# happyjin/Gaussian_process

Measured on AMD Instinct MI355X. Metric: GP-fit+predict sec and achieved fp64 TFLOP/s, N=65536 d=8, 1/2/4/8 MI355X, higher is better.
Workload: dtype f64; 1 GPU; GP fit+predict N=65536 d=8 n_test=4096 (BASELINE configs[2]); N=65536, d=8, n_test=4096, partition=single GPU

## Files before the change

### gaussian_process_amd/_lib.py

```python
from __future__ import annotations

import ctypes as C
import os

import numpy as np


_HERE = os.path.dirname(os.path.abspath(__file__))
LIB_PATH = os.path.join(_HERE, "libgpmi355x.so")

GPMI_OK, GPMI_ERR_NOT_PD, GPMI_ERR_BAD_ARG, GPMI_ERR_RUNTIME = 0, 1, 2, 3
ABI_VERSION = 4
SOFTMAX_MAX_CLASSES = 10
SPARSE_METHODS = {"vfe": 0, "fitc": 1}

T_KBUILD, T_CHOL, T_CHOL_PANEL, T_CHOL_TRAIL, T_LML, T_KS, T_SOLVE_V, T_MEANVAR, \
    T_ALPHA, T_POSTCHOL, T_TRAIL_LAUNCHES, T_TRAIL_FLOPS = range(12)
T_COUNT = 16
TIMER_NAMES = ["kbuild", "chol", "chol_panel", "chol_trail", "lml", "ks", "solve_v", "meanvar",
               "alpha", "postchol", "trail_launches", "trail_flops", "grad", "loo", "sparse"]

_dp = C.POINTER(C.c_double)
_i64 = C.c_int64
_vp = C.c_void_p

SIGNATURES = {
    "gpmi_abi_version": [],
    "gpmi_device_count": [C.POINTER(C.c_int)],
    "gpmi_ctx_create": [C.c_int, C.POINTER(_vp)],
    "gpmi_ctx_destroy": [_vp],
    "gpmi_set_option": [_vp, C.c_char_p, _i64],
    "gpmi_rbf": [_vp, _dp, _i64, _dp, _i64, _i64, C.c_double, C.c_double, _dp],
    "gpmi_cov": [_vp, C.c_int, _dp, _i64, _dp, _i64, _i64, C.c_double, C.c_double, _dp],
    "gpmi_set_kernel": [_vp, C.c_int, C.c_double, C.c_double],
    "gpmi_cov_params": [_vp, C.c_int, _dp, _i64, _dp, _i64, _i64, _dp, C.c_int, _dp],
    "gpmi_set_kernel_params": [_vp, C.c_int, _dp, C.c_int],
    "gpmi_set_train": [_vp, _dp, _i64, _i64, _dp],
    "gpmi_factorize": [_vp, C.c_double, C.c_double, C.c_double, _dp, C.POINTER(_i64)],
    "gpmi_fit": [_vp, _dp, _i64, _i64, _dp, C.c_double, C.c_double, C.c_double, _dp, C.POINTER(_i64)],
    "gpmi_append": [_vp, _dp, _i64, _dp, _dp, C.POINTER(_i64)],
    "gpmi_remove": [_vp, C.POINTER(_i64), _i64, _dp],
    "gpmi_get_layout": [_vp, C.POINTER(_i64)],
    "gpmi_get_alpha": [_vp, _dp],
    "gpmi_get_m": [_vp, _dp],
    "gpmi_get_diag": [_vp, _dp],
    "gpmi_get_factor_block": [_vp, _i64, _i64, _i64, _i64, _dp],
    "gpmi_set_test": [_vp, _dp, _i64],
    "gpmi_predict_resident": [_vp, _dp, _dp, C.c_int],
    "gpmi_predict": [_vp, _dp, _i64, _dp, _dp, C.c_int],
    "gpmi_fit_predict_resident": [_vp, C.c_double, C.c_double, C.c_double, _dp, C.POINTER(_i64), _dp, _dp, C.c_int],
    "gpmi_fit_predict_sample_resident": [_vp, C.c_double, C.c_double, C.c_double, C.c_double, _dp, C.POINTER(_i64), _dp, _dp,
                                         C.c_int, _dp],
    "gpmi_post_chol": [_vp, C.c_double, _dp, C.POINTER(_i64)],
    "gpmi_post_sample": [_vp, C.c_double, _dp, _i64, _dp, C.POINTER(_i64)],
    "gpmi_lml_grad": [_vp, _dp, _dp],
    "gpmi_set_lengthscales": [_vp, _dp, _i64],
    "gpmi_lml_grad_ard": [_vp, _dp, _dp, _dp, _dp],
    "gpmi_lml_grad_co2": [_vp, _dp, _dp],
    "gpmi_loo": [_vp, _dp, _dp, _dp, _dp],
    "gpmi_loo_grad": [_vp, _dp, _dp, _dp],
    "gpmi_grad_trace": [_vp, _dp, _dp, _i64, _i64, C.c_double, C.c_double, _dp, _dp, _dp, _dp],
    "gpmi_lml_batch": [_vp, _dp, _i64, _dp, C.POINTER(C.c_int)],
    "gpmi_laplace_fit": [_vp, C.c_double, C.c_double, C.c_double, C.c_int, _dp, C.POINTER(C.c_int), C.POINTER(C.c_int), _dp],
    "gpmi_laplace_predict_resident": [_vp, _dp, _dp, _dp],
    "gpmi_laplace_grad": [_vp, _dp, _dp, _dp],
# ... 118 lines not shown
```

### gaussian_process_amd/csrc/driver.hip

```cpp
#include "gpmi_ctx.h"
#include "gpmi_plan.h"

namespace gpmi {

hipError_t panel_rec(hipStream_t s, double* A, int64_t ld, int64_t mrows, int64_t off, int64_t w,
                     int64_t col_offset, int64_t* info) {
    hipError_t e;
    const bool fused = tuning().panel_fused && w % 128 == 0 && off % 128 == 0;
    const int64_t leaf = fused ? 128 : IB;
    if (w <= leaf) {
        double* Ajj = A + off * ld + off;
        const int64_t below = mrows - off - leaf;
        if (fused) {
            if ((e = launch_potrf128(s, Ajj, ld, col_offset + off, info)) != hipSuccess) return e;
            if (below > 0) return launch_trsm128(s, Ajj, ld, A + (off + leaf) * ld + off, ld, below);
            return hipSuccess;
        }
        if ((e = launch_potf2_64(s, Ajj, ld, col_offset + off, info)) != hipSuccess) return e;
        if (below > 0) return launch_trsm_rlt64(s, Ajj, ld, A + (off + IB) * ld + off, ld, below);
        return hipSuccess;
    }
    const int64_t h = (w / 2) / leaf * leaf;
    if ((e = panel_rec(s, A, ld, mrows, off, h, col_offset, info)) != hipSuccess) return e;
    {
// ... 12 lines not shown
}

hipError_t trsm_rec(hipStream_t s, const double* L, int64_t ldl, double* X, int64_t ldx, int64_t m,
                    int64_t off, int64_t w) {
    hipError_t e;
    const bool fused = tuning().panel_fused && w % 128 == 0 && off % 128 == 0 && m % 128 == 0;
    const int64_t leaf = fused ? 128 : IB;
    if (w <= leaf) {
        if (fused) return launch_trsm128(s, L + off * ldl + off, ldl, X + off, ldx, m);
        return launch_trsm_rlt64(s, L + off * ldl + off, ldl, X + off, ldx, m);
    }
    const int64_t h = (w / 2) / leaf * leaf;
    if ((e = trsm_rec(s, L, ldl, X, ldx, m, off, h)) != hipSuccess) return e;
    const GemmArgs g = gemm_minus(X + off + h, ldx, X + off, ldx, L + (off + h) * ldl + off, ldl, m, w - h, h);
    if ((e = launch_gemm_nt(s, g)) != hipSuccess) return e;
    return trsm_rec(s, L, ldl, X, ldx, m, off + h, w - h);
}

hipError_t trsm_block(hipStream_t s, const double* L, int64_t ldl, double* X, int64_t ldx,
                      int64_t m, int64_t nb) {
    return trsm_rec(s, L, ldl, X, ldx, m, 0, nb);
}

hipError_t cholesky_inplace(gpmi_ctx* c, double* A, int64_t ld, int64_t ncols, int64_t nrows,
                            int64_t* info, bool account, int64_t carried_rows) {
    hipError_t e;
    hipStream_t sm = c->stream;
    const int64_t NB = c->block(ncols);
    const bool la = c->lookahead_for(ncols);
    hipStream_t sp_ = la ? c->pstream : sm;
    const bool slack = la && ncols >= 49152;
    SharingScope shallow(la ? Sharing::beside_update().with_panel_slack(slack) : sharing());
    const int slot_p = account ? GPMI_T_CHOL_PANEL : GPMI_T_COUNT - 1;
    const int slot_t = account ? GPMI_T_CHOL_TRAIL : GPMI_T_COUNT - 1;
    if (la && (e = c->order(sm, sp_)) != hipSuccess) return e;
    auto trail = [&](hipStream_t st, bool counted, int64_t r0, int64_t c0, int64_t k, int64_t nb, int64_t ncol_upd) -> hipError_t {
        GemmArgs g = gemm_minus_lower(A + r0 * ld + c0, ld, A + r0 * ld + k, ld, A + c0 * ld + k, ld, nrows - r0, ncol_upd,
                                      nb, r0 - c0);
        g.role = counted ? 1 : 0;
        const GemmRoute route = gemm_nt_route(g);
        const bool dma = gemm_kernel_is_dma(route.kernel);
        size_t sp = c->span_begin(counted ? (dma ? slot_t : GPMI_T_COUNT - 1) : slot_p, st);
        hipError_t er = launch_gemm_nt(st, g, route);
        c->span_end(sp, st);
        if (account && dma && counted) {
            c->stage_ms[GPMI_T_TRAIL_LAUNCHES] += 1.0;
            c->stage_ms[GPMI_T_TRAIL_FLOPS] += gemm_nt_algorithmic_flops(g, ncols - r0 + 1 + carried_rows);
        }
        return er;
    };
    hipEvent_t ev_b = nullptr;
    for (int64_t k = 0; k < ncols; k += NB) {
        const int64_t nb = std::min<int64_t>(NB, ncols - k);
        size_t sp = c->span_begin(slot_p, sp_);
        {
            SharingScope panel_forms(!la ? sharing().large_lds()
                                     : (ncols - k >= c->shallow_min ? Sharing::beside_update() : Sharing::chip_shared_only()).with_panel_slack(slack));
            e = panel_factor(sp_, A + k * ld + k, ld, nb, nrows - k, k, info);
        }
        c->span_end(sp, sp_);
        if (e != hipSuccess) return e;
        if (la && (e = c->order(sp_, sm)) != hipSuccess) return e;
        const int64_t r0 = k + nb;
        if (r0 >= ncols) continue;
        if (!la) {
            if ((e = trail(sm, true, r0, r0, k, nb, ncols - r0)) != hipSuccess) return e;
            continue;
        }
        const int64_t nbn = std::min<int64_t>(NB, ncols - r0);
        if (ev_b && (e = hipStreamWaitEvent(sp_, ev_b, 0)) != hipSuccess) return e;
        if ((e = trail(sp_, false, r0, r0, k, nb, nbn)) != hipSuccess) return e;
        if (r0 + nbn < ncols) {
            if ((e = trail(sm, true, r0 + nbn, r0 + nbn, k, nb, ncols - r0 - nbn)) != hipSuccess) return e;
            ev_b = c->new_event();
            if (!ev_b) return c->ev_error;
            if ((e = hipEventRecord(ev_b, sm)) != hipSuccess) return e;
        }
    }
    return hipSuccess;
}

RbfArgs rbf_cross(const gpmi_ctx* c, const double* A, int64_t nA, const Box& ba, const double* B, int64_t nB, const Box& bb,
                  int64_t row0, int64_t nrows, int64_t ncols, double* out, int64_t ld) {
    RbfArgs r;
    r.A = A; r.B = B;
    r.nA = nA; r.nB = nB; r.d = c->d; r.row0 = row0; r.nrows = nrows; r.ncols = ncols;
    r.coef = c->coef; r.sig2 = c->sig2;
    r.kind = c->kind; r.kp0 = c->kp0; r.kp1 = c->kp1;
    for (int i = 0; i < 11; ++i) r.kpv[i] = c->kpv[i];
    r.diag_add = 0.; r.symmetric = 0;
    r.delta_square = (A == c->x_test() && B == c->x_train() && nA == nB) ? 1 : 0;
    r.max_sq = box_max_sq(ba, bb);
    r.out = out; r.ld = ld;
    return r;
}

RbfArgs rbf_sym(const gpmi_ctx* c, const double* X, int64_t n, const Box& box, double diag_add, int64_t npad, double* out,
                int64_t ld) {
    RbfArgs r = rbf_cross(c, X, n, box, X, n, box, 0, npad, npad, out, ld);
    r.diag_add = diag_add; r.symmetric = 1; r.delta_square = 1;
    return r;
}

RbfArgs rbf_test_train(const gpmi_ctx* c, double* out, int64_t ld) {
    return rbf_cross(c, c->x_test(), c->n, c->box_test(), c->x_train(), c->N, c->box_train(), 0, c->np_, c->Np, out, ld);
}

int ensure_train_buffers(gpmi_ctx* c, int64_t test_rows, bool test_cols) {
    c->spareA.release();
    c->Np = round_up(c->N, TILE);
    const int64_t cap = round_up(c->N + c->reserve, TILE);
    c->ldA = cap + (test_cols ? test_rows : 0) + c->ld_pad;
    c->Mp = c->Np + TILE + test_rows;
    c->rows_cap = cap + TILE + test_rows;
    c->yrow = test_cols ? c->Np + test_rows : c->Np;
    HIP_TRY(c->A.ensure((size_t)c->rows_cap * c->ldA * sizeof(double)));
    HIP_TRY(c->info.ensure(sizeof(int64_t)));
    HIP_TRY(c->red.ensure(16 * sizeof(double)));
    return GPMI_OK;
}

void meanvar_to_host(gpmi_ctx* c, const std::vector<double>& h, double* mu, double* out2, int want_sd) {
    for (int64_t i = 0; i < c->n; ++i) {
        if (mu) mu[i] = h[i];
        if (out2) {
            double kss = c->sig2;
            if (c->kind == 2) kss = 1.0;
            else if (c->kind == 3) {
                const double* th = c->kpv;
                kss = ((th[0] * th[0] + th[2] * th[2]) + th[5] * th[5]) + (th[8] * th[8] + th[10] * th[10]);
            }
            else if (c->kind == 1) {
                kss = 0.0;
                for (int64_t k = 0; k < c->d; ++k) {
                    const double e = c->hXs[(size_t)i * c->d + k] - c->kp0;
                    kss = kss + e * e;
                }
            }
            const double var = kss - h[c->np_ + i];
            out2[i] = want_sd ? std::sqrt(var) : var;
        }
    }
}

int factorize_impl(gpmi_ctx* c, double sigma, double ell, double noise_var, double* lml,
                   int64_t* bad_pivot, bool with_test, double* mu, double* out2, int want_sd, bool with_post, double jitter) {
    if (!c->res.have_train) return fail_arg("gpmi_factorize: no training set (call gpmi_set_train)");
    if (cov_stationary(c->kind) && (!(ell != 0.0) || std::isnan(ell) || std::isnan(sigma)))
        return fail_arg("gpmi_factorize: ell must be non-zero and hyper-parameters finite");
    if (std::isnan(noise_var)) return fail_arg("gpmi_factorize: noise_var is NaN");
    if (c->kind == 2 && c->d != 1) return fail_arg("gpmi_factorize: the periodic kernel is 1-D only (GP_regression.py:48)");
    if (!cov_stationary(c->kind) && c->ard())
        return fail_arg("gpmi_factorize: per-dimension lengthscales need the squared-exponential or a Matern kernel (kinds 0, 4, 5, 6)");
    if (with_post && std::isnan(jitter)) return fail_arg("gpmi_fit_predict_sample: jitter is NaN");
    c->res.drop_fit();
    c->release_sparse_grad();
    int rc = ensure_train_buffers(c, with_test ? c->np_ : 0, with_post);
    if (rc) return rc;
    hipStream_t s = c->stream;
    c->timers_reset({GPMI_T_KBUILD, GPMI_T_CHOL, GPMI_T_CHOL_PANEL, GPMI_T_CHOL_TRAIL, GPMI_T_LML,
                     GPMI_T_TRAIL_LAUNCHES, GPMI_T_TRAIL_FLOPS});
    if (with_test) c->timers_reset({GPMI_T_KS, GPMI_T_SOLVE_V, GPMI_T_MEANVAR});
    c->sig2 = sigma * sigma;
    c->coef = cov_coef(c->kind, ell);
    c->sigma = sigma; c->ell = ell; c->noise = noise_var;
    double* A = c->A.as<double>();
    const int64_t big = std::numeric_limits<int64_t>::max();
    HIP_TRY(hipMemcpyAsync(c->info.p, &big, sizeof big, hipMemcpyHostToDevice, s));

    size_t sp = c->span_begin(GPMI_T_KBUILD);
    const RbfArgs r = rbf_sym(c, c->x_train(), c->N, c->box_train(), noise_var, c->Np, A, c->ldA);
    HIP_TRY(launch_rbf(s, r));
    c->span_end(sp);
    const int64_t ncols = c->Np + (with_post ? c->np_ : 0);
    HIP_TRY(launch_fill_rows(s, c->m_row(), c->ldA, TILE, ncols, 0.0));
    HIP_TRY(launch_set_yrow(s, c->m_row(), c->y.as<double>(), c->N, c->Np));
    c->v_row0 = with_post ? c->Np : c->Np + TILE;
    double* Vr = A + c->v_row0 * c->ldA;
    if (with_test) {
        sp = c->span_begin(GPMI_T_KS);
        const RbfArgs t = rbf_test_train(c, Vr, c->ldA);
        HIP_TRY(launch_rbf(s, t));
        if (with_post) {
            const RbfArgs q = rbf_sym(c, c->x_test(), c->n, c->box_test(), jitter, c->np_, Vr + c->Np, c->ldA);
            HIP_TRY(launch_rbf(s, q));
        }
        c->span_end(sp);
    }

    sp = c->span_begin(GPMI_T_CHOL);
    HIP_TRY(cholesky_inplace(c, A, c->ldA, ncols, c->Mp, c->info.as<int64_t>(), true, with_test && !with_post ? c->n : 0));
    c->span_end(sp);

    sp = c->span_begin(GPMI_T_LML);
    HIP_TRY(launch_lml_reduce(s, A, c->ldA, c->m_row(), c->N, c->red.as<double>()));
    c->span_end(sp);

    std::vector<double> h;
    if (with_test) {
        HIP_TRY(c->vec.ensure((size_t)std::max(c->Np, c->np_) * 4 * 8));
        sp = c->span_begin(GPMI_T_MEANVAR);
        double* dot = c->vec.as<double>();
        HIP_TRY(launch_row_dots(s, Vr, c->ldA, c->np_, c->Np, c->m_row(), dot, dot + c->np_));
        c->span_end(sp);
        h.resize(2 * (size_t)c->np_);
        HIP_TRY(hipMemcpyAsync(h.data(), dot, h.size() * 8, hipMemcpyDeviceToHost, s));
    }
    double red[2];
    int64_t info;
    HIP_TRY(hipMemcpyAsync(red, c->red.p, sizeof red, hipMemcpyDeviceToHost, s));
    HIP_TRY(hipMemcpyAsync(&info, c->info.p, sizeof info, hipMemcpyDeviceToHost, s));
    HIP_TRY(hipStreamSynchronize(s));
    c->timers_collect();
    if (info != big && (info < c->N || (with_post && info >= c->Np && info < c->Np + c->n))) {
// ... 81 lines not shown
```

### gaussian_process_amd/csrc/gpmi_api.hip

```cpp
#include "gpmi_ctx.h"

using namespace gpmi;

namespace gpmi {
thread_local std::string g_err;

static thread_local Tuning t_dev_tuning;
static thread_local const Tuning* t_tuning = nullptr;
const Tuning& tuning() { return t_tuning ? *t_tuning : t_dev_tuning; }
TuneScope::TuneScope(const Tuning* t) : prev(t_tuning) { t_tuning = t; }
TuneScope::~TuneScope() { t_tuning = prev; }
static thread_local Sharing t_sharing;
Sharing& sharing() { return t_sharing; }

int ard_rescale_train(gpmi_ctx* c) {
    if (!c->ard()) return GPMI_OK;
    HIP_TRY(c->Xz.ensure((size_t)c->N * c->d * 8));
    HIP_TRY(launch_scale_inputs(c->stream, c->X.as<double>(), c->ard_rdev.as<double>(), c->N, c->d, c->Xz.as<double>()));
    HIP_TRY(hipStreamSynchronize(c->stream));
    box_scale(c->boxX, c->ard_r, c->boxZ);
    return GPMI_OK;
}
int ard_rescale_test(gpmi_ctx* c) {
    if (!c->ard()) return GPMI_OK;
// ... 37 lines not shown
    const char* env;
    if ((env = getenv("GPMI_NB"))) c->nb = std::max<int64_t>(128, atoll(env) / 128 * 128);
    if ((env = getenv("GPMI_LD_PAD"))) c->ld_pad = std::max<int64_t>(0, atoll(env) / 2 * 2);
    if ((env = getenv("GPMI_LOOKAHEAD"))) c->lookahead = atoi(env) ? 1 : 0;
    *out = c;
    return GPMI_OK;
}

int gpmi_ctx_destroy(gpmi_ctx* c) {
    if (!c) return GPMI_OK;
    for (gpmi_ctx* l : c->lane_ctx) (void)gpmi_ctx_destroy(l);
    c->lane_ctx.clear();
    (void)hipSetDevice(c->device);
    (void)hipStreamSynchronize(c->stream);
    for (DevBuf* b : {&c->X, &c->y, &c->A, &c->info, &c->red, &c->Xs, &c->V, &c->P, &c->vec, &c->dense,
                       &c->U, &c->Kn, &c->gpart, &c->cov_a, &c->cov_b, &c->cov_out, &c->flag, &c->vside,
                       &c->Xz, &c->Xsz, &c->ard_rdev, &c->gsum, &c->app, &c->spareA, &c->rem, &c->lap, &c->lap_part, &c->lap_out, &c->sm, &c->sm_part, &c->sm_E, &c->sm_B, &c->sm_out, &c->loov, &c->loow,
                       &c->sp_Zraw, &c->sp_Z, &c->sp_L, &c->sp_B, &c->sp_W, &c->sp_q, &c->sp_vec, &c->sp_part, &c->sp_scr, &c->sp_info, &c->sp_pred,
                       &c->sp_g0, &c->sp_g1, &c->sp_g2, &c->sp_gE, &c->sp_gpart, &c->sp_gvec})
        b->release();
    for (auto e : c->ev_pool) (void)hipEventDestroy(e);
    (void)hipStreamDestroy(c->stream);
    (void)hipStreamDestroy(c->pstream);
    delete c;
    return GPMI_OK;
}

static int set_tuning_option(Tuning& t, const char* name, int64_t value) {
    if (!strcmp(name, "gemm_small_tiles")) {
        t.gemm_small_tiles = value ? 1 : 0;
    } else if (!strcmp(name, "trsm_wave")) {
        t.trsm_wave = value ? 1 : 0;
    } else if (!strcmp(name, "gemm_small_dma")) {
        t.gemm_small_dma = value ? 1 : 0;
    } else if (!strcmp(name, "gemm_persist")) {
        t.gemm_persist = value ? 1 : 0;
    } else if (!strcmp(name, "gemm_ticket")) {
        if (value < 0 || value > 2) return fail_arg("gemm_ticket must be 0 (off), 1 (trailing updates under lookahead) or 2 (every launch)");
        t.gemm_ticket = (int)value;
    } else if (!strcmp(name, "gemm_balance")) {
        t.gemm_balance = value ? 1 : 0;
    } else if (!strcmp(name, "trsv_vinv")) {
        if (value < 0 || value > 2) return fail_arg("trsv_vinv must be 0 (16 x 16 rounds), 1 (one launch per block) or 2 (one launch)");
        t.trsv_vinv = (int)value;
    } else if (!strcmp(name, "panel_fused")) {
        t.panel_fused = value ? 1 : 0;
// ... 34 lines not shown
    } else if (!strcmp(name, "lookahead")) {
        c->lookahead = value ? 1 : 0;
    } else if (!strcmp(name, "la_min")) {
        if (value < 0) return fail_arg("la_min must be >= 0");
        c->la_min = value;
    } else if (!strcmp(name, "shallow_min")) {
        if (value < 0) return fail_arg("shallow_min must be >= 0");
        c->shallow_min = value;
    } else if (!strcmp(name, "sparse_slab")) {
        if (value < 0) return fail_arg("sparse_slab must be >= 0 (0: by size)");
        c->sparse_slab = value;
    } else if (!strcmp(name, "reserve")) {
        if (value < 0) return fail_arg("reserve must be >= 0 (points that gpmi_append may add in place)");
        c->reserve = value;
    } else if (!strcmp(name, "append_skinny")) {
        if (value < -1 || value > 1) return fail_arg("append_skinny must be -1 (by size), 0 (never) or 1 (whenever allowed)");
        c->append_skinny = (int)value;
    } else if (!strcmp(name, "remove_keep_spare")) {
        c->remove_keep_spare = value ? 1 : 0;
        if (!c->remove_keep_spare) {
            HIP_TRY(hipSetDevice(c->device));
            c->spareA.release();
        }
    } else if (!strcmp(name, "lanes")) {
        if (value < 0 || value > 8) return fail_arg("lanes must be 0 (by size) .. 8");
        c->lanes = (int)value;
    } else {
        const int rc = set_tuning_option(c->tune, name, value);
        if (rc < 0) return fail_arg("gpmi_set_option: unknown option");
        return rc;
    }
    return GPMI_OK;
}

int gpmi_dev_set_option(const char* name, int64_t value) {
    if (!name) return fail_arg("gpmi_dev_set_option: null argument");
    const int rc = set_tuning_option(t_dev_tuning, name, value);
    if (rc < 0) return fail_arg("gpmi_dev_set_option: unknown option");
    return rc;
}

int gpmi_set_kernel(gpmi_ctx* c, int kind, double p0, double p1) {
    if (!c) return fail_arg("gpmi_set_kernel: null context");
    if (kind < 0 || kind == 3 || kind > 6)
        return fail_arg("gpmi_set_kernel: kind must be 0 (rbf), 1 (linear), 2 (periodic) or 4, 5, 6 (Matern nu = 1/2, 3/2, 5/2)");
    if (kind == 2 && (!(p0 != 0.0) || !(p1 != 0.0))) return fail_arg("gpmi_set_kernel: period and lengthscale must be non-zero");
// ... 171 lines not shown
    const Tuning tn = resident_tuning(c);
    TuneScope tune_scope(&tn);
    return append_impl(c, Xnew, k, ynew, lml, bad_pivot);
}

int gpmi_remove(gpmi_ctx* c, const int64_t* idx, int64_t k, double* lml) {
    if (!c) return fail_arg("gpmi_remove: null context");
    HIP_TRY(hipSetDevice(c->device));
    const Tuning tn = resident_tuning(c);
    TuneScope tune_scope(&tn);
    return remove_impl(c, idx, k, lml);
}

int gpmi_get_layout(gpmi_ctx* c, int64_t* out5) {
    if (!c || !out5) return fail_arg("gpmi_get_layout: null argument");
    out5[0] = c->res.have_train ? c->N : 0;
    out5[1] = c->Np;
    out5[2] = c->ldA;
    out5[3] = c->rows_cap;
    out5[4] = c->append_route;
    return GPMI_OK;
}

int gpmi_get_m(gpmi_ctx* c, double* m_out) {
    if (!c || !m_out) return fail_arg("gpmi_get_m: null argument");
    if (!c->res.regression()) return fail_arg("gpmi_get_m: no factorisation resident");
    HIP_TRY(hipSetDevice(c->device));
    HIP_TRY(hipMemcpyAsync(m_out, c->m_row(), (size_t)c->N * 8,
                           hipMemcpyDeviceToHost, c->stream));
    HIP_TRY(hipStreamSynchronize(c->stream));
    return GPMI_OK;
}

int gpmi_get_diag(gpmi_ctx* c, double* diag_out) {
    if (!c || !diag_out) return fail_arg("gpmi_get_diag: null argument");
    if (!c->res.regression()) return fail_arg("gpmi_get_diag: no factorisation resident");
    HIP_TRY(hipSetDevice(c->device));
    HIP_TRY(hipMemcpy2DAsync(diag_out, 8, c->A.p, (size_t)(c->ldA + 1) * 8, 8, (size_t)c->N,
                             hipMemcpyDeviceToHost, c->stream));
    HIP_TRY(hipStreamSynchronize(c->stream));
    return GPMI_OK;
}

int gpmi_get_factor_block(gpmi_ctx* c, int64_t r0, int64_t r1, int64_t c0, int64_t c1, double* out) {
    if (!c || !out) return fail_arg("gpmi_get_factor_block: null argument");
    if (!c->res.regression()) return fail_arg("gpmi_get_factor_block: no factorisation resident");
// ... 112 lines not shown
int gpmi_grad_trace(gpmi_ctx* c, const double* a_in, const double* b_in, int64_t N, int64_t d, double sigma,
                    double ell, const double* alpha_in, const double* Kinv_in, double* d_ell, double* d_sigma) {
    if (!c || !a_in || !b_in || !alpha_in || !Kinv_in || !d_ell || !d_sigma) return fail_arg("gpmi_grad_trace: null argument");
    HIP_TRY(hipSetDevice(c->device));
    return grad_trace_impl(c, a_in, b_in, N, d, sigma, ell, alpha_in, Kinv_in, d_ell, d_sigma);
}

int gpmi_post_chol(gpmi_ctx* c, double jitter, double* L_out, int64_t* bad_pivot) {
    if (!c || !L_out) return fail_arg("gpmi_post_chol: null argument");
    HIP_TRY(hipSetDevice(c->device));
    TuneScope tune_scope(&c->tune);
    return post_chol_impl(c, jitter, L_out, bad_pivot);
}

int gpmi_post_sample(gpmi_ctx* c, double jitter, const double* Z, int64_t num_fun, double* LZ_out, int64_t* bad_pivot) {
    if (!c || !Z || !LZ_out) return fail_arg("gpmi_post_sample: null argument");
    HIP_TRY(hipSetDevice(c->device));
    TuneScope tune_scope(&c->tune);
    return post_sample_impl(c, jitter, Z, num_fun, LZ_out, bad_pivot);
}

static int lane_prepare(gpmi_ctx* c, gpmi_ctx* l) {
    l->nb = c->nb; l->ld_pad = c->ld_pad; l->lookahead = c->lookahead; l->la_min = c->la_min; l->timing = c->timing;
    l->tune = c->tune;
    l->kind = c->kind; l->kp0 = c->kp0; l->kp1 = c->kp1;
    for (int i = 0; i < 11; ++i) l->kpv[i] = c->kpv[i];
    l->N = c->N; l->d = c->d; l->boxX = c->box_train();
    HIP_TRY(l->X.ensure((size_t)c->N * c->d * 8));
    HIP_TRY(l->y.ensure((size_t)c->N * 8));
    HIP_TRY(hipMemcpyAsync(l->X.p, c->x_train(), (size_t)c->N * c->d * 8, hipMemcpyDeviceToDevice, l->stream));
    HIP_TRY(hipMemcpyAsync(l->y.p, c->y.p, (size_t)c->N * 8, hipMemcpyDeviceToDevice, l->stream));
    HIP_TRY(hipStreamSynchronize(l->stream));
    l->res.drop_train();
    l->res.train_set();
    return GPMI_OK;
}

int gpmi_lml_batch(gpmi_ctx* c, const double* triples, int64_t T, double* lml_out, int* status_out) {
    if (!c || !triples || !lml_out) return fail_arg("gpmi_lml_batch: null argument");
    if (T < 0) return fail_arg("gpmi_lml_batch: T < 0");
    if (!c->res.have_train) return fail_arg("gpmi_lml_batch: no training set (call gpmi_set_train)");
    HIP_TRY(hipSetDevice(c->device));
    const int64_t Np = round_up(c->N, TILE);
    int L = c->lanes ? c->lanes : (Np > 32768 ? 1 : Np >= 24576 ? 3 : Np >= 12288 ? 5 : 4);
    L = (int)std::min<int64_t>(L, std::max<int64_t>(T, 1));
    struct LaMinScope {
// ... 134 lines not shown
```

### gaussian_process_amd/csrc/gpmi_ctx.h

```cpp
#pragma once
#include <algorithm>
#include <cmath>
#include <cstdio>
#include <cstring>
#include <limits>
#include <string>
#include <thread>
#include <vector>

#include "../../include/gpmi.h"
#include "gpmi_internal.h"
#include "gpmi_state.h"

namespace gpmi {

extern thread_local std::string g_err;

inline int fail_runtime(hipError_t e, const char* what) {
    char buf[512];
    snprintf(buf, sizeof buf, "%s: %s (hipError %d)", what, hipGetErrorString(e), (int)e);
    g_err = buf;
    return GPMI_ERR_RUNTIME;
}
inline int fail_arg(const char* what) {
// ... 68 lines not shown
        out.hi[k] = raw.hi[k] / r[k];
    }
}
inline double box_max_sq(const Box& a, const Box& b) {
    if (!a.valid || !b.valid || a.lo.size() != b.lo.size()) return -1.0;
    double s = 0.0;
    for (size_t k = 0; k < a.lo.size(); ++k) {
        const double w = std::max(a.hi[k] - b.lo[k], b.hi[k] - a.lo[k]);
        s += w * w;
    }
    return std::isfinite(s) ? s : -1.0;
}

}

using gpmi::Box;
using gpmi::DevBuf;
using gpmi::TimedSpan;

struct gpmi_ctx {
    int device = 0;
    hipStream_t stream = nullptr;
    hipStream_t pstream = nullptr;
    int64_t nb = 0;
    int64_t block(int64_t ncols) const { return nb ? nb : (ncols >= 32768 ? 2048 : ncols >= 12288 ? 1024 : 512); }
    int64_t ld_pad = 544;
    int timing = 1;
    int lookahead = 1;
    int64_t la_min = 6144;
    int64_t shallow_min = 6144;
    bool lookahead_for(int64_t ncols) const { return lookahead && pstream && ncols > block(ncols) && ncols >= la_min; }
    int lanes = 0;
    std::vector<gpmi_ctx*> lane_ctx;
    int64_t reserve = 0;
    int append_route = -1;
    int append_skinny = -1;
    gpmi::Tuning tune;
    int64_t N = 0, d = 0, Np = 0, ldA = 0, Mp = 0;
    int64_t rows_cap = 0;
    gpmi::Resident res;
    double sig2 = 1.0, coef = -0.5;
    int kind = 0;
    double kp0 = 0., kp1 = 0.;
    double kpv[11] = {0., 0., 0., 0., 0., 0., 0., 0., 0., 0., 0.};
    DevBuf X, y, A, info, red;
    int64_t n = 0, np_ = 0, ldV = 0, ldP = 0;
    int64_t v_row0 = 0;
    double* v_rows() { return res.v_in_A ? A.as<double>() + v_row0 * ldA : V.as<double>(); }
    int64_t yrow = 0;
    double* m_row() { return A.as<double>() + yrow * ldA; }
    std::vector<double> hXs;
    Box boxX, boxXs;
    std::vector<double> ard_r;
    DevBuf Xz, Xsz, ard_rdev;
    Box boxZ, boxZs;
    bool ard() const { return !ard_r.empty(); }
    const double* x_train() const { return ard() ? Xz.as<double>() : X.as<double>(); }
    const double* x_test() const { return ard() ? Xsz.as<double>() : Xs.as<double>(); }
    const Box& box_train() const { return ard() ? boxZ : boxX; }
    const Box& box_test() const { return ard() ? boxZs : boxXs; }
    DevBuf Xs, V, P, vec, dense;
    DevBuf flag;
    DevBuf vside;
    DevBuf cov_a, cov_b, cov_out;
    DevBuf U, Kn, gpart;
    DevBuf gsum;
    double sigma = 1.0, ell = 1.0;
    double noise = 0.0;
    DevBuf app;
    int remove_keep_spare = 0;
    DevBuf spareA, rem;
    DevBuf loov, loow;
// ... 24 lines not shown
        }
        return ev_pool[ev_used++];
    }
    static constexpr size_t NO_SPAN = (size_t)-1;
    size_t span_begin(int slot, hipStream_t st = nullptr) {
        if (!timing) return NO_SPAN;
        TimedSpan s{new_event(), new_event(), slot};
        if (!s.a || !s.b) return NO_SPAN;
        if (hipEventRecord(s.a, st ? st : stream) != hipSuccess) return NO_SPAN;
        spans.push_back(s);
        return spans.size() - 1;
    }
    void span_end(size_t idx, hipStream_t st = nullptr) {
        if (!timing || idx == NO_SPAN) return;
        if (hipEventRecord(spans[idx].b, st ? st : stream) != hipSuccess) spans[idx].slot = GPMI_T_COUNT - 1;
    }
    hipError_t order(hipStream_t signaller, hipStream_t waiter) {
        hipEvent_t e = new_event();
        if (!e) return ev_error;
        hipError_t r = hipEventRecord(e, signaller);
        if (r != hipSuccess) return r;
        return hipStreamWaitEvent(waiter, e, 0);
    }
    void timers_reset(std::initializer_list<int> slots) {
        for (int s : slots) stage_ms[s] = 0.;
    }
    void timers_collect() {
        for (auto& s : spans) {
            float ms = 0.f;
            if (hipEventElapsedTime(&ms, s.a, s.b) == hipSuccess) stage_ms[s.slot] += ms;
        }
        spans.clear();
        ev_used = 0;
    }
};


namespace gpmi {

hipError_t panel_factor(hipStream_t s, double* A, int64_t ld, int64_t nb, int64_t mrows, int64_t col_offset,
                        int64_t* info);
hipError_t trsm_block(hipStream_t s, const double* L, int64_t ldl, double* X, int64_t ldx, int64_t m, int64_t nb);
hipError_t cholesky_inplace(gpmi_ctx* c, double* A, int64_t ld, int64_t ncols, int64_t nrows, int64_t* info,
                            bool account, int64_t carried_rows = 0);
hipError_t solve_sweep(gpmi_ctx* c, double* V, int64_t ldv, int64_t m, bool tri = false);
hipError_t solve_sweep_factor(gpmi_ctx* c, const double* L, int64_t ld, int64_t ncols, double* V, int64_t ldv, int64_t m,
                              bool tri = false);
hipError_t inverse_transposed(gpmi_ctx* c, const double* F, int64_t ldf, int64_t n, double* V, int64_t ldv);
hipError_t neg_gram_lower(gpmi_ctx* c, const double* V, double* Out, int64_t ld, int64_t n);
hipError_t neg_gram_lower_dense(gpmi_ctx* c, const double* V, double* Out, int64_t ld, int64_t n);
RbfArgs rbf_cross(const gpmi_ctx* c, const double* A, int64_t nA, const Box& ba, const double* B, int64_t nB, const Box& bb,
                  int64_t row0, int64_t nrows, int64_t ncols, double* out, int64_t ld);
RbfArgs rbf_sym(const gpmi_ctx* c, const double* X, int64_t n, const Box& box, double diag_add, int64_t npad, double* out,
                int64_t ld);
RbfArgs rbf_test_train(const gpmi_ctx* c, double* out, int64_t ld);
int ensure_train_buffers(gpmi_ctx* c, int64_t test_rows = 0, bool test_cols = false);
int append_impl(gpmi_ctx* c, const double* Xnew, int64_t k, const double* ynew, double* lml, int64_t* bad_pivot);
int remove_impl(gpmi_ctx* c, const int64_t* idx, int64_t k, double* lml);
int factorize_impl(gpmi_ctx* c, double sigma, double ell, double noise_var, double* lml, int64_t* bad_pivot,
                   bool with_test = false, double* mu = nullptr, double* out2 = nullptr, int want_sd = 1,
                   bool with_post = false, double jitter = 0.0);
int ard_rescale_train(gpmi_ctx* c);
int ard_rescale_test(gpmi_ctx* c);
void meanvar_to_host(gpmi_ctx* c, const std::vector<double>& h, double* mu, double* out2, int want_sd);
hipError_t backward_solve_fused(gpmi_ctx* c, double* b, double* xout);
hipError_t backward_solve_resident(gpmi_ctx* c, double* x2, double** x_out);
hipError_t backward_solve_rhs(gpmi_ctx* c, double* x2, double** x_out);
int fail_gave_up(const char* api);
int alpha_impl(gpmi_ctx* c, double* alpha_out);
int factor_inverse_front(gpmi_ctx* c, int slot, bool want_kn, double** alpha_out, size_t* span);
int grad_ard_finish(gpmi_ctx* c, GradArdArgs& a, size_t span, const char* solve_api, std::vector<double>* sums);
void grad_ard_scale(const gpmi_ctx* c, const GradArdArgs& a, const std::vector<double>& sums, double l2, double* d_r,
                    double* d_ell, double* d_sigma, double* d_noise);
int predict_front(gpmi_ctx* c, int ks_slot);
int predict_resident_impl(gpmi_ctx* c, double* mu, double* out2, int want_sd);
int lml_grad_impl(gpmi_ctx* c, double* d_ell, double* d_sigma);
int lml_grad_ard_impl(gpmi_ctx* c, double* d_r, double* d_ell, double* d_sigma, double* d_noise);
int lml_grad_co2_impl(gpmi_ctx* c, double* d_theta, double* d_noise);
int loo_impl(gpmi_ctx* c, double* mu, double* var, double* logp, double* loo);
// ... 43 lines not shown
```

### gaussian_process_amd/csrc/gpmi_internal.h

```cpp
#pragma once
#include <hip/hip_runtime.h>
#include <stdint.h>

#include <cmath>
#include <mutex>

#include "gpmi_kroute.h"
#include "gpmi_route.h"

namespace gpmi {

constexpr int TILE = 128;
constexpr int IB = 64;

struct Tuning : GemmTuning {
    int trsm_wave = 1;
    int rbf_blocks = 16384;
    int trsv_vinv = 2;
    int panel_fused = 1;
    unsigned long long* gemm_stamps = nullptr;
    unsigned long long* panel_stamps = nullptr;
};
const Tuning& tuning();
struct TuneScope {
// ... 54 lines not shown
    g.lower = 1; g.diag_off = diag_off;
    return g;
}
GemmRoute gemm_nt_route(const GemmArgs& a);
hipError_t launch_gemm_nt(hipStream_t s, const GemmArgs& a, const GemmRoute& r);
inline hipError_t launch_gemm_nt(hipStream_t s, const GemmArgs& a) { return launch_gemm_nt(s, a, gemm_nt_route(a)); }
double gemm_nt_algorithmic_flops(const GemmArgs& a, int64_t real_rows);
hipError_t launch_gemm_nt_dma(hipStream_t s, const GemmArgs& a, const GemmRoute& r);
hipError_t launch_gemm_nt_small(hipStream_t s, const GemmArgs& a, const GemmRoute& r);
int gemm_resident_groups();
double gemm_nt_flops(const GemmArgs& a);

hipError_t launch_potf2_64(hipStream_t s, double* A, int64_t ld, int64_t col_offset,
                           int64_t* info_dev);
hipError_t launch_trsm_rlt64(hipStream_t s, const double* L, int64_t ldl, double* X, int64_t ldx,
                             int64_t m);

hipError_t launch_potrf128(hipStream_t s, double* A, int64_t ld, int64_t col_offset, int64_t* info_dev);

hipError_t launch_trsm128(hipStream_t s, const double* L, int64_t ldl, double* X, int64_t ldx, int64_t m);

hipError_t launch_border_sweep(hipStream_t s, const double* L, int64_t ldl, int64_t ncols, double* X, int64_t ldx,
                               int64_t rows);

struct RbfArgs {
    const double* A;
    const double* B;
    int64_t nA, nB, d;
    int64_t row0;
    int64_t nrows;
    int64_t ncols;
    double coef;
    double sig2;
    double diag_add;
    int symmetric;
    double* out;
    int64_t ld;
    int kind = 0;
    double kp0 = 0., kp1 = 0.;
    double kpv[11] = {0., 0., 0., 0., 0., 0., 0., 0., 0., 0., 0.};
    int delta_square = 0;
    int64_t delta_col0 = 0;
    double max_sq = -1.0;
};
hipError_t launch_rbf(hipStream_t s, const RbfArgs& a);
inline int cov_family(int kind) { return rbf_family(kind); }
// ... 106 lines not shown
```

### gaussian_process_amd/csrc/panel_mfma.hip

```cpp
#include "gpmi_internal.h"
#include <utility>

namespace gpmi {

typedef double d4 __attribute__((ext_vector_type(4)));
typedef double d2 __attribute__((ext_vector_type(2)));

namespace {

constexpr int PB = 128;
constexpr int NT = PB / 16;
constexpr int TILE_BYTES = 16 * 128;
constexpr int NTILES = NT * (NT + 1) / 2;
constexpr int POTRF_TILES = NT + 1;
constexpr int TRSM_ROWS = 64;
constexpr int SCR_LD = 18;

__device__ __forceinline__ int kap(int g, int v) { return 2 * g + (v & 1) + 8 * (v >> 1); }
__device__ __forceinline__ int rho_inv(int n) { return ((n >> 1) & 3) + 4 * (n & 1) + 8 * (n >> 3); }

__device__ __forceinline__ double readlane_d(double v, int lane) {
    int lo = __double2loint(v), hi = __double2hiint(v);
    lo = __builtin_amdgcn_readlane(lo, lane);
    hi = __builtin_amdgcn_readlane(hi, lane);
// ... 531 lines not shown
    return hipGetLastError();
}

hipError_t launch_trsm128(hipStream_t s, const double* L, int64_t ldl, double* X, int64_t ldx, int64_t m) {
    if (m <= 0) return hipSuccess;
    if (m % TRSM_ROWS || ldl % 2 || ldx % 2 || (reinterpret_cast<uintptr_t>(L) & 15) || (reinterpret_cast<uintptr_t>(X) & 15))
        return hipErrorInvalidValue;
    hipError_t e = panel_mfma_attrs();
    if (e != hipSuccess) return e;
    const int64_t nslabs = m / TRSM_ROWS;
    const unsigned grid = (unsigned)std::min<int64_t>(nslabs, 512);
    if (sharing().small_lds) {
        hipLaunchKernelGGL(trsm128_kernel<0>, dim3(grid), dim3(256), trsm_tiles<0>() * TILE_BYTES, s, L, ldl, X, ldx, nslabs,
                           tuning().panel_stamps);
        hipLaunchKernelGGL(trsm128_kernel<1>, dim3(grid), dim3(256), trsm_tiles<1>() * TILE_BYTES, s, L, ldl, X, ldx, nslabs,
                           tuning().panel_stamps);
        return hipGetLastError();
    }
    hipLaunchKernelGGL(trsm128_kernel<-1>, dim3(grid), dim3(256), NTILES * TILE_BYTES, s, L, ldl, X, ldx, nslabs,
                       tuning().panel_stamps);
    return hipGetLastError();
}

hipError_t launch_border_sweep(hipStream_t s, const double* L, int64_t ldl, int64_t ncols, double* X, int64_t ldx,
                               int64_t rows) {
    if (rows < 1 || rows > 16 || ncols < 0 || ncols % PB || ldl % 2 || ldx % 2 || ldl < ncols || ldx < ncols ||
        (reinterpret_cast<uintptr_t>(L) & 15) || (reinterpret_cast<uintptr_t>(X) & 15))
        return hipErrorInvalidValue;
    if (ncols == 0) return hipSuccess;
    hipError_t e = panel_mfma_attrs();
    if (e != hipSuccess) return e;
    const int64_t nblk = ncols / PB;
    for (int64_t t = 0; t < nblk; ++t)
        hipLaunchKernelGGL(border_sweep_kernel, dim3((unsigned)(nblk - t)), dim3(256), SWEEP_LDS, s, L, ldl, X, ldx, (int)rows, t);
    return hipGetLastError();
}

hipError_t launch_vinv128(hipStream_t s, double* A, int64_t ld, int64_t n, double* vside) {
    if (n <= 0 || n % PB || ld % 2 || (reinterpret_cast<uintptr_t>(A) & 15) || (reinterpret_cast<uintptr_t>(vside) & 15))
        return hipErrorInvalidValue;
    hipError_t e = panel_mfma_attrs();
    if (e != hipSuccess) return e;
    if (vside) {
        e = hipMemsetAsync(vside, 0, (size_t)n * PB * sizeof(double), s);
        if (e != hipSuccess) return e;
    }
    hipLaunchKernelGGL(vinv128_kernel, dim3((unsigned)(n / PB)), dim3(256), NTILES * TILE_BYTES, s, A, ld, vside);
    return hipGetLastError();
}

}
```

### gaussian_process_amd/gp.py

```python
from __future__ import annotations

import ctypes as C
import threading

import numpy as np

from . import _lib
from ._lib import as_f64, check, ptr, scalar


def softmax_labels(labels, n_classes=None):
    lab = as_f64(labels, 1, "labels")
    if lab.size == 0 or not np.all(np.isfinite(lab)) or np.any(lab != np.floor(lab)):
        raise ValueError("labels must be integers in [0, n_classes)")
    if n_classes is None:
        n_classes = int(lab.max()) + 1
    if n_classes != int(n_classes) or not 2 <= int(n_classes) <= _lib.SOFTMAX_MAX_CLASSES:
        raise ValueError("n_classes must be an integer in [2, %d], got %r" % (_lib.SOFTMAX_MAX_CLASSES, n_classes))
    n_classes = int(n_classes)
    if lab.min() < 0 or lab.max() >= n_classes:
        raise ValueError("labels must be integers in [0, n_classes = %d)" % n_classes)
    return lab, n_classes


# ... 197 lines not shown
        st = self._lib.gpmi_append(self._h, ptr(Xnew), Xnew.shape[0], ptr(ynew), C.byref(lml), C.byref(bad))
        if st != _lib.GPMI_ERR_BAD_ARG:
            self.N = self.layout()["N"]
        check(st, bad.value)
        return lml.value

    def remove(self, idx):
        idx = np.ascontiguousarray(np.asarray(idx).reshape(-1))
        if idx.size and not np.issubdtype(idx.dtype, np.integer):
            raise ValueError("idx must hold integers, got dtype %s" % idx.dtype)
        idx = np.ascontiguousarray(idx, dtype=np.int64)
        lml = C.c_double()
        st = self._lib.gpmi_remove(self._h, idx.ctypes.data_as(C.POINTER(C.c_int64)), idx.shape[0], C.byref(lml))
        if st != _lib.GPMI_ERR_BAD_ARG:
            self.N = self.layout()["N"]
        check(st)
        return lml.value

    def layout(self):
        out = (C.c_int64 * 5)()
        check(self._lib.gpmi_get_layout(self._h, out))
        return dict(zip(("N", "Np", "ld", "rows", "route"), (int(v) for v in out)))

    def alpha(self):
        out = np.empty(self.N)
        check(self._lib.gpmi_get_alpha(self._h, ptr(out)))
        return out

    def m(self):
        out = np.empty(self.N)
        check(self._lib.gpmi_get_m(self._h, ptr(out)))
        return out

    def diag(self):
        out = np.empty(self.N)
        check(self._lib.gpmi_get_diag(self._h, ptr(out)))
        return out

    def factor(self, r0=0, r1=None, c0=0, c1=None):
        r1 = self.N if r1 is None else r1
        c1 = self.N if c1 is None else c1
        out = np.empty((r1 - r0, c1 - c0))
        check(self._lib.gpmi_get_factor_block(self._h, r0, r1, c0, c1, ptr(out)))
        return out

    def set_test(self, Xs):
# ... 238 lines not shown
```

### include/gpmi.h

```cpp
#ifndef GPMI_H
#define GPMI_H

#include <stdint.h>

#ifdef __cplusplus
extern "C" {
#endif

#define GPMI_OK 0
#define GPMI_ERR_NOT_PD 1
#define GPMI_ERR_BAD_ARG 2
#define GPMI_ERR_RUNTIME 3

#define GPMI_ABI_VERSION 4

enum {
    GPMI_T_KBUILD = 0,
    GPMI_T_CHOL = 1,
    GPMI_T_CHOL_PANEL = 2,
    GPMI_T_CHOL_TRAIL = 3,
    GPMI_T_LML = 4,
    GPMI_T_KS = 5,
    GPMI_T_SOLVE_V = 6,
    GPMI_T_MEANVAR = 7,
// ... 18 lines not shown
int gpmi_set_option(gpmi_ctx* ctx, const char* name, int64_t value);

int gpmi_rbf(gpmi_ctx* ctx, const double* a, int64_t N, const double* b, int64_t M,
             int64_t d, double sigma, double ell, double* out);

int gpmi_cov(gpmi_ctx* ctx, int kind, const double* a, int64_t N, const double* b, int64_t M,
             int64_t d, double p0, double p1, double* out);
int gpmi_set_kernel(gpmi_ctx* ctx, int kind, double p0, double p1);
int gpmi_cov_params(gpmi_ctx* ctx, int kind, const double* a, int64_t N, const double* b, int64_t M,
                    int64_t d, const double* params, int nparams, double* out);
int gpmi_set_kernel_params(gpmi_ctx* ctx, int kind, const double* params, int nparams);

int gpmi_set_train(gpmi_ctx* ctx, const double* X, int64_t N, int64_t d, const double* y);

int gpmi_factorize(gpmi_ctx* ctx, double sigma, double ell, double noise_var,
                   double* lml, int64_t* bad_pivot);

int gpmi_fit(gpmi_ctx* ctx, const double* X, int64_t N, int64_t d, const double* y,
             double sigma, double ell, double noise_var, double* lml, int64_t* bad_pivot);

int gpmi_append(gpmi_ctx* ctx, const double* Xnew, int64_t k, const double* ynew, double* lml, int64_t* bad_pivot);
int gpmi_remove(gpmi_ctx* ctx, const int64_t* idx, int64_t k, double* lml);
int gpmi_get_layout(gpmi_ctx* ctx, int64_t* out5);

int gpmi_get_alpha(gpmi_ctx* ctx, double* alpha_out);
int gpmi_get_m(gpmi_ctx* ctx, double* m_out);
int gpmi_get_diag(gpmi_ctx* ctx, double* diag_out);
int gpmi_get_factor_block(gpmi_ctx* ctx, int64_t r0, int64_t r1, int64_t c0, int64_t c1,
                          double* out);

int gpmi_set_test(gpmi_ctx* ctx, const double* Xs, int64_t n);

int gpmi_predict_resident(gpmi_ctx* ctx, double* mu, double* out2, int want_sd);
int gpmi_predict(gpmi_ctx* ctx, const double* Xs, int64_t n, double* mu, double* out2,
                 int want_sd);

int gpmi_fit_predict_resident(gpmi_ctx* ctx, double sigma, double ell, double noise_var, double* lml, int64_t* bad_pivot,
                              double* mu, double* out2, int want_sd);

int gpmi_fit_predict_sample_resident(gpmi_ctx* ctx, double sigma, double ell, double noise_var, double jitter, double* lml,
                                     int64_t* bad_pivot, double* mu, double* out2, int want_sd, double* L_out);

int gpmi_post_chol(gpmi_ctx* ctx, double jitter, double* L_out, int64_t* bad_pivot);

int gpmi_post_sample(gpmi_ctx* ctx, double jitter, const double* Z, int64_t num_fun, double* LZ_out, int64_t* bad_pivot);

// ... 115 lines not shown
```

Baseline: 69.24 TFLOP/s.

## Sweep the y row on a side stream behind each Cholesky panel

```diff
diff --git a/gaussian_process_amd/_lib.py b/gaussian_process_amd/_lib.py
--- a/gaussian_process_amd/_lib.py
+++ b/gaussian_process_amd/_lib.py
@@ -41,6 +41,7 @@
     "gpmi_append": [_vp, _dp, _i64, _dp, _dp, C.POINTER(_i64)],
     "gpmi_remove": [_vp, C.POINTER(_i64), _i64, _dp],
     "gpmi_get_layout": [_vp, C.POINTER(_i64)],
+    "gpmi_get_y_row": [_vp, C.POINTER(_i64)],
     "gpmi_get_alpha": [_vp, _dp],
     "gpmi_get_m": [_vp, _dp],
     "gpmi_get_diag": [_vp, _dp],
diff --git a/gaussian_process_amd/csrc/driver.hip b/gaussian_process_amd/csrc/driver.hip
--- a/gaussian_process_amd/csrc/driver.hip
+++ b/gaussian_process_amd/csrc/driver.hip
@@ -1,5 +1,6 @@
 #include "gpmi_ctx.h"
 #include "gpmi_plan.h"
+#include "gpmi_ysweep.h"
 
 namespace gpmi {
 
@@ -58,10 +59,25 @@
     return trsm_rec(s, L, ldl, X, ldx, m, 0, nb);
 }
 
+static hipError_t cholesky_steps(gpmi_ctx* c, double* A, int64_t ld, int64_t ncols, int64_t nrows, int64_t* info,
+                                 bool account, int64_t carried_rows, double* y_swept);
+
 hipError_t cholesky_inplace(gpmi_ctx* c, double* A, int64_t ld, int64_t ncols, int64_t nrows,
-                            int64_t* info, bool account, int64_t carried_rows) {
+                            int64_t* info, bool account, int64_t carried_rows, double* y_swept) {
+    if (y_swept && !c->ystream) return hipErrorInvalidValue;
+    hipError_t e = cholesky_steps(c, A, ld, ncols, nrows, info, account, carried_rows, y_swept);
+    if (y_swept) {
+        const hipError_t j = c->order(c->ystream, c->stream);
+        if (e == hipSuccess) e = j;
+    }
+    return e;
+}
+
+static hipError_t cholesky_steps(gpmi_ctx* c, double* A, int64_t ld, int64_t ncols, int64_t nrows, int64_t* info,
+                                 bool account, int64_t carried_rows, double* y_swept) {
     hipError_t e;
     hipStream_t sm = c->stream;
+    const YSweepSchedule ys = y_swept ? ysweep_schedule(ncols, c->block(ncols)) : YSweepSchedule();
     const int64_t NB = c->block(ncols);
     const bool la = c->lookahead_for(ncols);
     hipStream_t sp_ = la ? c->pstream : sm;
@@ -81,12 +97,13 @@
         c->span_end(sp, st);
         if (account && dma && counted) {
             c->stage_ms[GPMI_T_TRAIL_LAUNCHES] += 1.0;
-            c->stage_ms[GPMI_T_TRAIL_FLOPS] += gemm_nt_algorithmic_flops(g, ncols - r0 + 1 + carried_rows);
+            c->stage_ms[GPMI_T_TRAIL_FLOPS] += gemm_nt_algorithmic_flops(g, ncols - r0 + (y_swept ? 0 : 1) + carried_rows);
         }
         return er;
     };
     hipEvent_t ev_b = nullptr;
-    for (int64_t k = 0; k < ncols; k += NB) {
+    int64_t step = 0;
+    for (int64_t k = 0; k < ncols; k += NB, ++step) {
         const int64_t nb = std::min<int64_t>(NB, ncols - k);
         size_t sp = c->span_begin(slot_p, sp_);
         {
@@ -96,7 +113,18 @@
         }
         c->span_end(sp, sp_);
         if (e != hipSuccess) return e;
-        if (la && (e = c->order(sp_, sm)) != hipSuccess) return e;
+        if (la || y_swept) {
+            hipEvent_t ev_p = c->new_event();
+            if (!ev_p) return c->ev_error;
+            if ((e = hipEventRecord(ev_p, sp_)) != hipSuccess) return e;
+            if (la && (e = hipStreamWaitEvent(sm, ev_p, 0)) != hipSuccess) return e;
+            if (y_swept) {
+                const YSweepStep& st = ys.steps[(size_t)step];
+                if ((e = hipStreamWaitEvent(c->ystream, ev_p, 0)) != hipSuccess) return e;
+                if ((e = launch_border_sweep_range(c->ystream, A, ld, ncols, y_swept, ld, 1, st.range.t0, st.range.t1)) != hipSuccess)
+                    return e;
+            }
+        }
         const int64_t r0 = k + nb;
         if (r0 >= ncols) continue;
         if (!la) {
@@ -142,14 +170,15 @@
     return rbf_cross(c, c->x_test(), c->n, c->box_test(), c->x_train(), c->N, c->box_train(), 0, c->np_, c->Np, out, ld);
 }
 
-int ensure_train_buffers(gpmi_ctx* c, int64_t test_rows, bool test_cols) {
+int ensure_train_buffers(gpmi_ctx* c, int64_t test_rows, bool test_cols, bool y_swept) {
     c->spareA.release();
     c->Np = round_up(c->N, TILE);
     const int64_t cap = round_up(c->N + c->reserve, TILE);
     c->ldA = cap + (test_cols ? test_rows : 0) + c->ld_pad;
     c->Mp = c->Np + TILE + test_rows;
     c->rows_cap = cap + TILE + test_rows;
-    c->yrow = test_cols ? c->Np + test_rows : c->Np;
+    c->yrow = test_cols || y_swept ? c->Np + test_rows : c->Np;
+    c->y_swept = y_swept;
     HIP_TRY(c->A.ensure((size_t)c->rows_cap * c->ldA * sizeof(double)));
     HIP_TRY(c->info.ensure(sizeof(int64_t)));
     HIP_TRY(c->red.ensure(16 * sizeof(double)));
@@ -191,7 +220,10 @@
     if (with_post && std::isnan(jitter)) return fail_arg("gpmi_fit_predict_sample: jitter is NaN");
     c->res.drop_fit();
     c->release_sparse_grad();
-    int rc = ensure_train_buffers(c, with_test ? c->np_ : 0, with_post);
+    const int64_t fcols = round_up(c->N, TILE) + (with_post ? c->np_ : 0);
+    const bool swept = ysweep_applies(c->y_sweep, tuning().panel_fused != 0, c->lookahead_for(fcols), fcols, c->block(fcols));
+    if (swept) HIP_TRY(c->ensure_ystream());
+    int rc = ensure_train_buffers(c, with_test ? c->np_ : 0, with_post, swept);
     if (rc) return rc;
     hipStream_t s = c->stream;
     c->timers_reset({GPMI_T_KBUILD, GPMI_T_CHOL, GPMI_T_CHOL_PANEL, GPMI_T_CHOL_TRAIL, GPMI_T_LML,
@@ -211,7 +243,7 @@
     const int64_t ncols = c->Np + (with_post ? c->np_ : 0);
     HIP_TRY(launch_fill_rows(s, c->m_row(), c->ldA, TILE, ncols, 0.0));
     HIP_TRY(launch_set_yrow(s, c->m_row(), c->y.as<double>(), c->N, c->Np));
-    c->v_row0 = with_post ? c->Np : c->Np + TILE;
+    c->v_row0 = with_post || swept ? c->Np : c->Np + TILE;
     double* Vr = A + c->v_row0 * c->ldA;
     if (with_test) {
         sp = c->span_begin(GPMI_T_KS);
@@ -225,7 +257,8 @@
     }
 
     sp = c->span_begin(GPMI_T_CHOL);
-    HIP_TRY(cholesky_inplace(c, A, c->ldA, ncols, c->Mp, c->info.as<int64_t>(), true, with_test && !with_post ? c->n : 0));
+    HIP_TRY(cholesky_inplace(c, A, c->ldA, ncols, swept ? c->Mp - TILE : c->Mp, c->info.as<int64_t>(), true,
+                             with_test && !with_post ? c->n : 0, swept ? c->m_row() : nullptr));
     c->span_end(sp);
 
     sp = c->span_begin(GPMI_T_LML);
diff --git a/gaussian_process_amd/csrc/gpmi_api.hip b/gaussian_process_amd/csrc/gpmi_api.hip
--- a/gaussian_process_amd/csrc/gpmi_api.hip
+++ b/gaussian_process_amd/csrc/gpmi_api.hip
@@ -83,6 +83,7 @@
     for (auto e : c->ev_pool) (void)hipEventDestroy(e);
     (void)hipStreamDestroy(c->stream);
     (void)hipStreamDestroy(c->pstream);
+    if (c->ystream) (void)hipStreamDestroy(c->ystream);
     delete c;
     return GPMI_OK;
 }
@@ -163,6 +164,9 @@
             HIP_TRY(hipSetDevice(c->device));
             c->spareA.release();
         }
+    } else if (!strcmp(name, "y_sweep")) {
+        if (value < 0 || value > 2) return fail_arg("y_sweep must be 0 (the y row rides), 1 (swept where the panel chain has slack) or 2 (swept whenever the factor allows)");
+        c->y_sweep = (int)value;
     } else if (!strcmp(name, "lanes")) {
         if (value < 0 || value > 8) return fail_arg("lanes must be 0 (by size) .. 8");
         c->lanes = (int)value;
@@ -380,6 +384,14 @@
     return GPMI_OK;
 }
 
+int gpmi_get_y_row(gpmi_ctx* c, int64_t* out2) {
+    if (!c || !out2) return fail_arg("gpmi_get_y_row: null argument");
+    if (!c->res.regression()) return fail_arg("gpmi_get_y_row: no factorisation resident");
+    out2[0] = c->yrow;
+    out2[1] = c->y_swept ? 1 : 0;
+    return GPMI_OK;
+}
+
 int gpmi_get_m(gpmi_ctx* c, double* m_out) {
     if (!c || !m_out) return fail_arg("gpmi_get_m: null argument");
     if (!c->res.regression()) return fail_arg("gpmi_get_m: no factorisation resident");
@@ -538,6 +550,7 @@
 
 static int lane_prepare(gpmi_ctx* c, gpmi_ctx* l) {
     l->nb = c->nb; l->ld_pad = c->ld_pad; l->lookahead = c->lookahead; l->la_min = c->la_min; l->timing = c->timing;
+    l->y_sweep = c->y_sweep;
     l->tune = c->tune;
     l->kind = c->kind; l->kp0 = c->kp0; l->kp1 = c->kp1;
     for (int i = 0; i < 11; ++i) l->kpv[i] = c->kpv[i];
diff --git a/gaussian_process_amd/csrc/gpmi_ctx.h b/gaussian_process_amd/csrc/gpmi_ctx.h
--- a/gaussian_process_amd/csrc/gpmi_ctx.h
+++ b/gaussian_process_amd/csrc/gpmi_ctx.h
@@ -114,6 +114,7 @@
     int device = 0;
     hipStream_t stream = nullptr;
     hipStream_t pstream = nullptr;
+    hipStream_t ystream = nullptr;
     int64_t nb = 0;
     int64_t block(int64_t ncols) const { return nb ? nb : (ncols >= 32768 ? 2048 : ncols >= 12288 ? 1024 : 512); }
     int64_t ld_pad = 544;
@@ -122,6 +123,7 @@
     int64_t la_min = 6144;
     int64_t shallow_min = 6144;
     bool lookahead_for(int64_t ncols) const { return lookahead && pstream && ncols > block(ncols) && ncols >= la_min; }
+    int y_sweep = 1;
     int lanes = 0;
     std::vector<gpmi_ctx*> lane_ctx;
     int64_t reserve = 0;
@@ -140,6 +142,7 @@
     int64_t v_row0 = 0;
     double* v_rows() { return res.v_in_A ? A.as<double>() + v_row0 * ldA : V.as<double>(); }
     int64_t yrow = 0;
+    bool y_swept = false;
     double* m_row() { return A.as<double>() + yrow * ldA; }
     std::vector<double> hXs;
     Box boxX, boxXs;
@@ -210,6 +213,12 @@
         if (r != hipSuccess) return r;
         return hipStreamWaitEvent(waiter, e, 0);
     }
+    hipError_t ensure_ystream() {
+        if (ystream) return hipSuccess;
+        int prio_lo = 0, prio_hi = 0;
+        (void)hipDeviceGetStreamPriorityRange(&prio_lo, &prio_hi);
+        return hipStreamCreateWithPriority(&ystream, hipStreamNonBlocking, prio_lo);
+    }
     void timers_reset(std::initializer_list<int> slots) {
         for (int s : slots) stage_ms[s] = 0.;
     }
@@ -230,7 +239,7 @@
                         int64_t* info);
 hipError_t trsm_block(hipStream_t s, const double* L, int64_t ldl, double* X, int64_t ldx, int64_t m, int64_t nb);
 hipError_t cholesky_inplace(gpmi_ctx* c, double* A, int64_t ld, int64_t ncols, int64_t nrows, int64_t* info,
-                            bool account, int64_t carried_rows = 0);
+                            bool account, int64_t carried_rows = 0, double* y_swept = nullptr);
 hipError_t solve_sweep(gpmi_ctx* c, double* V, int64_t ldv, int64_t m, bool tri = false);
 hipError_t solve_sweep_factor(gpmi_ctx* c, const double* L, int64_t ld, int64_t ncols, double* V, int64_t ldv, int64_t m,
                               bool tri = false);
@@ -242,7 +251,7 @@
 RbfArgs rbf_sym(const gpmi_ctx* c, const double* X, int64_t n, const Box& box, double diag_add, int64_t npad, double* out,
                 int64_t ld);
 RbfArgs rbf_test_train(const gpmi_ctx* c, double* out, int64_t ld);
-int ensure_train_buffers(gpmi_ctx* c, int64_t test_rows = 0, bool test_cols = false);
+int ensure_train_buffers(gpmi_ctx* c, int64_t test_rows = 0, bool test_cols = false, bool y_swept = false);
 int append_impl(gpmi_ctx* c, const double* Xnew, int64_t k, const double* ynew, double* lml, int64_t* bad_pivot);
 int remove_impl(gpmi_ctx* c, const int64_t* idx, int64_t k, double* lml);
 int factorize_impl(gpmi_ctx* c, double sigma, double ell, double noise_var, double* lml, int64_t* bad_pivot,
diff --git a/gaussian_process_amd/csrc/gpmi_internal.h b/gaussian_process_amd/csrc/gpmi_internal.h
--- a/gaussian_process_amd/csrc/gpmi_internal.h
+++ b/gaussian_process_amd/csrc/gpmi_internal.h
@@ -100,6 +100,8 @@
 
 hipError_t launch_border_sweep(hipStream_t s, const double* L, int64_t ldl, int64_t ncols, double* X, int64_t ldx,
                                int64_t rows);
+hipError_t launch_border_sweep_range(hipStream_t s, const double* L, int64_t ldl, int64_t ncols, double* X, int64_t ldx,
+                                     int64_t rows, int64_t t0, int64_t t1);
 
 struct RbfArgs {
     const double* A;
diff --git a/gaussian_process_amd/csrc/gpmi_ysweep.h b/gaussian_process_amd/csrc/gpmi_ysweep.h
--- /dev/null
+++ b/gaussian_process_amd/csrc/gpmi_ysweep.h
@@ -0,0 +1,57 @@
+#pragma once
+#include <stdint.h>
+
+#include <algorithm>
+#include <vector>
+
+namespace gpmi {
+
+constexpr int YSWEEP_BLOCK = 128;
+constexpr int64_t YSWEEP_MIN_COLS = 49152;
+
+inline bool ysweep_applies(int option, bool fused, bool lookahead, int64_t ncols, int64_t outer_block) {
+    if (option <= 0 || !fused || ncols <= 0 || ncols % YSWEEP_BLOCK || outer_block % YSWEEP_BLOCK) return false;
+    return option >= 2 || (lookahead && ncols >= YSWEEP_MIN_COLS);
+}
+
+struct YSweepRange {
+    int64_t t0 = 0, t1 = 0;
+};
+inline YSweepRange ysweep_behind_panel(int64_t k, int64_t nb) {
+    YSweepRange r;
+    r.t0 = k / YSWEEP_BLOCK;
+    r.t1 = (k + nb) / YSWEEP_BLOCK;
+    return r;
+}
+
+struct YSweepStep {
+    int64_t panel = 0;
+    int64_t k = 0, nb = 0;
+    YSweepRange range;
+    int64_t wait_panel = 0;
+    int64_t after_sweep = -1;
+};
+struct YSweepSchedule {
+    int64_t nblk = 0;
+    std::vector<YSweepStep> steps;
+    bool end_joins = false;
+};
+inline YSweepSchedule ysweep_schedule(int64_t ncols, int64_t outer_block) {
+    YSweepSchedule s;
+    s.nblk = ncols / YSWEEP_BLOCK;
+    int64_t i = 0;
+    for (int64_t k = 0; k < ncols; k += outer_block, ++i) {
+        YSweepStep st;
+        st.panel = i;
+        st.k = k;
+        st.nb = std::min<int64_t>(outer_block, ncols - k);
+        st.range = ysweep_behind_panel(st.k, st.nb);
+        st.wait_panel = i;
+        st.after_sweep = i - 1;
+        s.steps.push_back(st);
+    }
+    s.end_joins = !s.steps.empty();
+    return s;
+}
+
+}
diff --git a/gaussian_process_amd/csrc/panel_mfma.hip b/gaussian_process_amd/csrc/panel_mfma.hip
--- a/gaussian_process_amd/csrc/panel_mfma.hip
+++ b/gaussian_process_amd/csrc/panel_mfma.hip
@@ -577,18 +577,24 @@
     return hipGetLastError();
 }
 
-hipError_t launch_border_sweep(hipStream_t s, const double* L, int64_t ldl, int64_t ncols, double* X, int64_t ldx,
-                               int64_t rows) {
+hipError_t launch_border_sweep_range(hipStream_t s, const double* L, int64_t ldl, int64_t ncols, double* X, int64_t ldx,
+                                     int64_t rows, int64_t t0, int64_t t1) {
     if (rows < 1 || rows > 16 || ncols < 0 || ncols % PB || ldl % 2 || ldx % 2 || ldl < ncols || ldx < ncols ||
         (reinterpret_cast<uintptr_t>(L) & 15) || (reinterpret_cast<uintptr_t>(X) & 15))
         return hipErrorInvalidValue;
-    if (ncols == 0) return hipSuccess;
+    const int64_t nblk = ncols / PB;
+    if (t0 < 0 || t1 < t0 || t1 > nblk) return hipErrorInvalidValue;
+    if (t0 == t1) return hipSuccess;
     hipError_t e = panel_mfma_attrs();
     if (e != hipSuccess) return e;
-    const int64_t nblk = ncols / PB;
-    for (int64_t t = 0; t < nblk; ++t)
+    for (int64_t t = t0; t < t1; ++t)
         hipLaunchKernelGGL(border_sweep_kernel, dim3((unsigned)(nblk - t)), dim3(256), SWEEP_LDS, s, L, ldl, X, ldx, (int)rows, t);
     return hipGetLastError();
+}
+
+hipError_t launch_border_sweep(hipStream_t s, const double* L, int64_t ldl, int64_t ncols, double* X, int64_t ldx,
+                               int64_t rows) {
+    return launch_border_sweep_range(s, L, ldl, ncols, X, ldx, rows, 0, ncols / PB);
 }
 
 hipError_t launch_vinv128(hipStream_t s, double* A, int64_t ld, int64_t n, double* vside) {
diff --git a/gaussian_process_amd/gp.py b/gaussian_process_amd/gp.py
--- a/gaussian_process_amd/gp.py
+++ b/gaussian_process_amd/gp.py
@@ -243,6 +243,11 @@
         check(self._lib.gpmi_get_layout(self._h, out))
         return dict(zip(("N", "Np", "ld", "rows", "route"), (int(v) for v in out)))
 
+    def y_row(self):
+        out = (C.c_int64 * 2)()
+        check(self._lib.gpmi_get_y_row(self._h, out))
+        return int(out[0]), bool(out[1])
+
     def alpha(self):
         out = np.empty(self.N)
         check(self._lib.gpmi_get_alpha(self._h, ptr(out)))
diff --git a/include/gpmi.h b/include/gpmi.h
--- a/include/gpmi.h
+++ b/include/gpmi.h
@@ -64,6 +64,7 @@
 int gpmi_append(gpmi_ctx* ctx, const double* Xnew, int64_t k, const double* ynew, double* lml, int64_t* bad_pivot);
 int gpmi_remove(gpmi_ctx* ctx, const int64_t* idx, int64_t k, double* lml);
 int gpmi_get_layout(gpmi_ctx* ctx, int64_t* out5);
+int gpmi_get_y_row(gpmi_ctx* ctx, int64_t* out2);
 
 int gpmi_get_alpha(gpmi_ctx* ctx, double* alpha_out);
 int gpmi_get_m(gpmi_ctx* ctx, double* m_out);
```

After: 69.49 TFLOP/s, median of 6. About the same (+0.4%).
